# jcorsetti/oryon

Measured on AMD Instinct MI355X. Metric: image-pairs/sec end-to-end (feat+match+reg) @224², C=256; ADD(-S) parity, higher is better.
Workload: dtype f32

## Files before the change

oryon_amd/csrc/pdsc_encoder.hip:

```cpp
#include <stdlib.h>
#include "common.h"
#include "pdsc.h"
#include "pdsc_blocks.h"

namespace oryon {

__global__ __launch_bounds__(256) void pdsc_center_kernel(const float *__restrict__ src, const float *__restrict__ tgt,
                                                           const int32_t *__restrict__ n_rows, int n_cap,
                                                           float *__restrict__ corr_pos )
{
    __shared__ double s_part[4][6];
    __shared__ float s_mean[6];
    const int b = blockIdx.x, t = threadIdx.x, lane = t & 63, wave = t >> 6;
    const int n = n_rows[b];
    const float *s = src + (size_t)b * n_cap * 3, *g = tgt + (size_t)b * n_cap * 3;
    double acc[6] = {0, 0, 0, 0, 0, 0};
    for (int i = t; i < n; i += 256) {
#pragma unroll
        for (int d = 0; d < 3; ++d) { acc[d] += s[3 * i + d]; acc[3 + d] += g[3 * i + d]; }
    }
#pragma unroll
    for (int d = 0; d < 6; ++d) {
        double v = acc[d];
#pragma unroll
        for (int off = 32; off > 0; off >>= 1) v += __shfl_xor(v, off);
        if (lane == 0) s_part[wave][d] = v;
    }
    __syncthreads();
    if (t < 6) s_mean[t] = (float)((s_part[0][t] + s_part[1][t] + s_part[2][t] + s_part[3][t]) / (double)(n > 0 ? n : 1));
    __syncthreads();
    float *o = corr_pos + (size_t)b * n_cap * 8;
    for (int i = t; i < n_cap; i += 256) {
        float v[8];
#pragma unroll
        for (int d = 0; d < 3; ++d) {
            v[d] = i < n ? s[3 * i + d] - s_mean[d] : 0.0f;
            v[3 + d] = i < n ? g[3 * i + d] - s_mean[3 + d] : 0.0f;
        }
        v[6] = v[7] = 0.0f;
#pragma unroll
        for (int d = 0; d < 8; ++d) o[(size_t)i * 8 + d] = v[d];
    }
}

constexpr int LIN_ROWS = 64, LIN_COLS = 128, LIN_BK = 32, LIN_LD = LIN_BK + 1;

template <bool RELU, bool RESID>
__global__ __launch_bounds__(256) void pdsc_linear_kernel(const float *__restrict__ X, int ldx, size_t x_batch,
                                                           const float *__restrict__ W, const float *__restrict__ bias,
                                                           const float *__restrict__ R, int ldr, size_t r_batch,
                                                           float *__restrict__ Y, int ldy, size_t y_batch, int K, int N,
                                                           const int32_t *__restrict__ n_rows)
{
    __shared__ float Xs[LIN_ROWS * LIN_LD];
    __shared__ float Ws[LIN_COLS * LIN_LD];
    const int b = blockIdx.z;
    const int m0 = blockIdx.x * LIN_ROWS, n0 = blockIdx.y * LIN_COLS;
    if (n_rows && m0 >= n_rows[b]) return;
    const int t = threadIdx.x, lane = t & 63, wave = t >> 6;
    const int wm = wave >> 1, wn = wave & 1, l31 = lane & 31, hi = lane >> 5;
    const float *x = X + (size_t)b * x_batch + (size_t)m0 * ldx;
    f32x16 acc[2];
#pragma unroll
    for (int j = 0; j < 2; ++j)
#pragma unroll
        for (int r = 0; r < 16; ++r) acc[j][r] = 0.0f;

    for (int k0 = 0; k0 < K; k0 += LIN_BK) {
        constexpr int NX = (LIN_ROWS * LIN_BK) / 256, NW = (LIN_COLS * LIN_BK) / 256;
        float xv[NX], wv[NW];
#pragma unroll
        for (int i = 0; i < NX; ++i) {
            const int e = t + 256 * i, row = e >> 5, kk = e & 31;
            xv[i] = (k0 + kk < K) ? x[(size_t)row * ldx + k0 + kk] : 0.0f;
        }
#pragma unroll
        for (int i = 0; i < NW; ++i) {
            const int e = t + 256 * i, col = e >> 5, kk = e & 31;
            wv[i] = (n0 + col < N && k0 + kk < K) ? W[(size_t)(n0 + col) * K + k0 + kk] : 0.0f;
        }
        __syncthreads();
#pragma unroll
        for (int i = 0; i < NX; ++i) {
            const int e = t + 256 * i;
            Xs[(e >> 5) * LIN_LD + (e & 31)] = xv[i];
        }
#pragma unroll
        for (int i = 0; i < NW; ++i) {
            const int e = t + 256 * i;
            Ws[(e >> 5) * LIN_LD + (e & 31)] = wv[i];
        }
        __syncthreads();
        const float *xa = Xs + (wm * 32 + l31) * LIN_LD + hi;
        const float *wb = Ws + (wn * 64 + l31) * LIN_LD + hi;
#pragma unroll
        for (int ks = 0; ks < LIN_BK / 2; ++ks) {
            const float a = xa[2 * ks];
            acc[0] = __builtin_amdgcn_mfma_f32_32x32x2f32(a, wb[2 * ks], acc[0], 0, 0, 0);
            acc[1] = __builtin_amdgcn_mfma_f32_32x32x2f32(a, wb[32 * LIN_LD + 2 * ks], acc[1], 0, 0, 0);
        }
    }
#pragma unroll
    for (int j = 0; j < 2; ++j) {
        const int c = n0 + wn * 64 + j * 32 + l31;
        if (c >= N) continue;
        const float bv = bias ? bias[c] : 0.0f;
#pragma unroll
        for (int r = 0; r < 16; ++r) {
            const int row = m0 + wm * 32 + crow(r, hi);
            float v = acc[j][r] + bv;
            if (RELU) v = v > 0.0f ? v : 0.0f;
            if (RESID) v += R[(size_t)b * r_batch + (size_t)row * ldr + c];
            Y[(size_t)b * y_batch + (size_t)row * ldy + c] = v;
        }
    }
}

__global__ __launch_bounds__(256) void pdsc_sc_kernel(const float *__restrict__ src, const float *__restrict__ tgt,
                                                       const int32_t *__restrict__ n_rows, int n_cap, float inv_sigma2,
                                                       float *__restrict__ sc)
{
    const int b = blockIdx.z, kt = blockIdx.y;
    const int n = n_rows[b];
    const int t = threadIdx.x, lane = t & 63, wave = t >> 6, l31 = lane & 31, hi = lane >> 5;
    const int qb = blockIdx.x * 4 + wave;
    if (qb * 32 >= n || kt * ATT_KT >= n) return;
    const float *sp = src + (size_t)b * n_cap * 3, *tp = tgt + (size_t)b * n_cap * 3;
    const int q = qb * 32 + l31;
    float sq[3], tq[3];
#pragma unroll
    for (int d = 0; d < 3; ++d) { sq[d] = sp[(size_t)q * 3 + d]; tq[d] = tp[(size_t)q * 3 + d]; }
    float4 *out = reinterpret_cast<float4 *>(sc) + ((((size_t)b * (n_cap / 32) + qb) * (n_cap / ATT_KT) + kt) * 8) * 64 + lane;
#pragma unroll
    for (int v4 = 0; v4 < 8; ++v4) {
        float o[4];
#pragma unroll
        for (int e = 0; e < 4; ++e) {
            const int r = (v4 & 3) * 4 + e, kb = v4 >> 2;
            const int k = kt * ATT_KT + kb * 32 + crow(r, hi);
            float v = -1.0f;
            if (k < n) {
                const float dx = sq[0] - sp[(size_t)k * 3], dy = sq[1] - sp[(size_t)k * 3 + 1], dz = sq[2] - sp[(size_t)k * 3 + 2];
                const float ex = tq[0] - tp[(size_t)k * 3], ey = tq[1] - tp[(size_t)k * 3 + 1], ez = tq[2] - tp[(size_t)k * 3 + 2];
                const float ds = sqrt_rn(dx * dx + dy * dy + dz * dz);
                const float dt = sqrt_rn(ex * ex + ey * ey + ez * ez);
                const float df = ds - dt;
                v = 1.0f - df * df * inv_sigma2;
                v = v > 0.0f ? v : 0.0f;
            }
            o[e] = v;
        }
        out[(size_t)v4 * 64] = make_float4(o[0], o[1], o[2], o[3]);
    }
}

template <int C>
__global__ __launch_bounds__(256) void pdsc_attention_kernel(const float *__restrict__ QKV, const float *__restrict__ sc,
                                                              const int32_t *__restrict__ n_rows, int n_cap,
                                                              float inv_sqrt_c, float *__restrict__ msg,
                                                              int KS, float *__restrict__ part_o, float *__restrict__ part_ml)
{
    constexpr int LD = C + 4;
    constexpr int CB = C / 32;
    constexpr int F4_PER_ROW = C / 4, PER_THREAD = ATT_KT * F4_PER_ROW / 256;
    __shared__ __attribute__((aligned(16))) float Ks[ATT_KT * LD];
    __shared__ __attribute__((aligned(16))) float Vs[ATT_KT * LD];
    const int b = blockIdx.z, split = blockIdx.y;
    const int n = n_rows[b];
    const int q0 = blockIdx.x * ATT_Q;
    if (q0 >= n) return;
    const int n_tiles = (n + ATT_KT - 1) / ATT_KT, per = (n_tiles + KS - 1) / KS;
    const int j_begin = split * per * ATT_KT;
    const int j_end = ((split + 1) * per * ATT_KT < n) ? (split + 1) * per * ATT_KT : n;
    const int t = threadIdx.x, lane = t & 63, wave = t >> 6, l31 = lane & 31, hi = lane >> 5;
    const int qrow = q0 + wave * 32 + l31;
    const float *base = QKV + (size_t)b * n_cap * 3 * C;
    const float4 *sc_q = reinterpret_cast<const float4 *>(sc) + (((size_t)b * (n_cap / 32) + (q0 / 32 + wave)) * (n_cap / ATT_KT)) * 8 * 64 + lane;
    const bool q_live = q0 + wave * 32 < n;

    float4 kv[PER_THREAD], vv[PER_THREAD], scv[8];
    auto fetch = [&](int j0) {
#pragma unroll
        for (int i = 0; i < PER_THREAD; ++i) {
            const int e = t + 256 * i, row = e / F4_PER_ROW, c4 = e % F4_PER_ROW;
            const bool in = j0 + row < n_cap;
            const float *rp = base + (size_t)(in ? j0 + row : 0) * 3 * C;
            kv[i] = in ? *reinterpret_cast<const float4 *>(rp + C + 4 * c4) : make_float4(0.f, 0.f, 0.f, 0.f);
            vv[i] = in ? *reinterpret_cast<const float4 *>(rp + 2 * C + 4 * c4) : make_float4(0.f, 0.f, 0.f, 0.f);
        }
        const float4 *sp = sc_q + (size_t)(j0 / ATT_KT) * 8 * 64;
#pragma unroll
        for (int v4 = 0; v4 < 8; ++v4) scv[v4] = q_live ? sp[(size_t)v4 * 64] : make_float4(-1.f, -1.f, -1.f, -1.f);
    };
    auto land = [&]() {
#pragma unroll
        for (int i = 0; i < PER_THREAD; ++i) {
            const int e = t + 256 * i, row = e / F4_PER_ROW, c4 = e % F4_PER_ROW;
            *reinterpret_cast<float4 *>(Ks + row * LD + 4 * c4) = kv[i];
            *reinterpret_cast<float4 *>(Vs + row * LD + 4 * c4) = vv[i];
        }
    };

    float qreg[C / 2];
    {
        const float2 *qv = reinterpret_cast<const float2 *>(base + (size_t)qrow * 3 * C);
#pragma unroll
        for (int ks = 0; ks < C / 2; ++ks) {
            const float2 v = qv[ks];
            qreg[ks] = hi ? v.y : v.x;
        }
    }
    f32x16 acc_o[CB];
#pragma unroll
    for (int cb = 0; cb < CB; ++cb)
#pragma unroll
        for (int r = 0; r < 16; ++r) acc_o[cb][r] = 0.0f;
    float m_run = -INFINITY, l_run = 0.0f;

    if (j_begin < j_end) fetch(j_begin);
    for (int j0 = j_begin; j0 < j_end; j0 += ATT_KT) {
        __syncthreads();
        land();
        float4 sct[8];
#pragma unroll
        for (int v4 = 0; v4 < 8; ++v4) sct[v4] = scv[v4];
        __syncthreads();
        if (j0 + ATT_KT < j_end) fetch(j0 + ATT_KT);

        f32x16 s[2];
#pragma unroll
        for (int kb = 0; kb < 2; ++kb)
#pragma unroll
            for (int r = 0; r < 16; ++r) s[kb][r] = 0.0f;
        {
            const float *ka0 = Ks + l31 * LD + hi, *ka1 = Ks + (32 + l31) * LD + hi;
#pragma unroll
            for (int ks = 0; ks < C / 2; ++ks) {
                s[0] = __builtin_amdgcn_mfma_f32_32x32x2f32(ka0[2 * ks], qreg[ks], s[0], 0, 0, 0);
                s[1] = __builtin_amdgcn_mfma_f32_32x32x2f32(ka1[2 * ks], qreg[ks], s[1], 0, 0, 0);
            }
        }
        float m_tile = -INFINITY;
#pragma unroll
        for (int kb = 0; kb < 2; ++kb)
#pragma unroll
            for (int r = 0; r < 16; ++r) {
                const float4 q4 = sct[kb * 4 + (r >> 2)];
                const float scq = (r & 3) == 0 ? q4.x : (r & 3) == 1 ? q4.y : (r & 3) == 2 ? q4.z : q4.w;
                float v = scq * (s[kb][r] * inv_sqrt_c);
                v = (scq >= 0.0f) ? v : -INFINITY;
                s[kb][r] = v;
                m_tile = fmaxf(m_tile, v);
            }
        m_tile = fmaxf(m_tile, __shfl_xor(m_tile, 32));
        const float m_new = fmaxf(m_run, m_tile);
        const float alpha = __expf(m_run - m_new);
        float l_tile = 0.0f;
#pragma unroll
        for (int kb = 0; kb < 2; ++kb)
#pragma unroll
            for (int r = 0; r < 16; ++r) {
                const float p = expf(s[kb][r] - m_new);
                s[kb][r] = p;
                l_tile += p;
            }
        l_run = l_run * alpha + l_tile;
        m_run = m_new;
#pragma unroll
        for (int cb = 0; cb < CB; ++cb)
#pragma unroll
            for (int r = 0; r < 16; ++r) acc_o[cb][r] *= alpha;
#pragma unroll
        for (int kb = 0; kb < 2; ++kb)
#pragma unroll
            for (int r = 0; r < 16; ++r) {
                const float *va = Vs + (kb * 32 + crow(r, hi)) * LD + l31;
                const float p = s[kb][r];
#pragma unroll
                for (int cb = 0; cb < CB; ++cb) acc_o[cb] = __builtin_amdgcn_mfma_f32_32x32x2f32(va[cb * 32], p, acc_o[cb], 0, 0, 0);
            }
    }
    const float l_all = l_run + __shfl_xor(l_run, 32);
    if (KS > 1) {
        const size_t prow = ((size_t)split * gridDim.z + b) * n_cap + qrow;
        float *po = part_o + prow * C;
#pragma unroll
        for (int cb = 0; cb < CB; ++cb)
#pragma unroll
            for (int g = 0; g < 4; ++g) {
                float4 v;
                v.x = acc_o[cb][4 * g + 0]; v.y = acc_o[cb][4 * g + 1]; v.z = acc_o[cb][4 * g + 2]; v.w = acc_o[cb][4 * g + 3];
                *reinterpret_cast<float4 *>(po + cb * 32 + 8 * g + 4 * hi) = v;
            }
        if (hi == 0) { part_ml[prow * 2] = m_run; part_ml[prow * 2 + 1] = l_all; }
        return;
    }
// ... 1325 lines not shown
```

oryon_amd/csrc/pdsc_solver.hip:

```cpp
#include <stdlib.h>
#include "common.h"
#include "kabsch.h"
#include "pdsc.h"

namespace oryon {

__global__ __launch_bounds__(256) void pdsc_seed_keys_kernel(const float *__restrict__ src, const float *__restrict__ conf,
                                                              const int32_t *__restrict__ n_rows, int n_cap, float radius,
                                                              float *__restrict__ key)
{
    extern __shared__ float sm[];
    float *px = sm, *py = sm + n_cap, *pz = sm + 2 * n_cap, *sc = sm + 3 * n_cap;
    const int b = blockIdx.y, t = threadIdx.x;
    const int n = n_rows[b];
    if ((int)blockIdx.x * 64 >= n) return;
    for (int i = t; i < n; i += 256) {
        px[i] = src[((size_t)b * n_cap + i) * 3 + 0];
        py[i] = src[((size_t)b * n_cap + i) * 3 + 1];
        pz[i] = src[((size_t)b * n_cap + i) * 3 + 2];
        sc[i] = conf[(size_t)b * n_cap + i];
    }
    __syncthreads();
    const int i = blockIdx.x * 64 + (t >> 2), part = t & 3;
    bool lm = true;
// ... 323 lines not shown
        const float4 *fa = reinterpret_cast<const float4 *>(kf + a * (C + 4)), *fb = reinterpret_cast<const float4 *>(kf + c2 * (C + 4));
        for (int c4 = 0; c4 < C / 4; ++c4) {
            const float4 x = fa[c4], y = fb[c4];
            dot = fmaf(x.x, y.x, dot);
            dot = fmaf(x.y, y.y, dot);
            dot = fmaf(x.z, y.z, dot);
            dot = fmaf(x.w, y.w, dot);
        }
        float fm = 1.0f - (1.0f - dot) * inv_sigma2;
        fm = fm > 0.0f ? fm : 0.0f;
        const float *pa = kc + a * 6, *pb = kc + c2 * 6;
        const float dx = pa[0] - pb[0], dy = pa[1] - pb[1], dz = pa[2] - pb[2];
        const float ex = pa[3] - pb[3], ey = pa[4] - pb[4], ez = pa[5] - pb[5];
        const float df = sqrt_rn(dx * dx + dy * dy + dz * dz) - sqrt_rn(ex * ex + ey * ey + ez * ez);
        float smv = 1.0f - df * df * inv_sigma_d2;
        smv = smv > 0.0f ? smv : 0.0f;
        const float v = fm * smv;
        Mo[a * k_cfg + c2] = v;
        Mo[c2 * k_cfg + a] = v;
    }
}

__device__ __forceinline__ unsigned wave_min_u32(unsigned v)
{
#define ORYON_DPP_MIN(ctrl, rmask)                                                                                              \
    {                                                                                                                           \
        const unsigned o = (unsigned)__builtin_amdgcn_update_dpp((int)v, (int)v, ctrl, rmask, 0xf, false);                      \
        v = o < v ? o : v;                                                                                                      \
    }
    ORYON_DPP_MIN(0x111, 0xf)
    ORYON_DPP_MIN(0x112, 0xf)
    ORYON_DPP_MIN(0x114, 0xf)
    ORYON_DPP_MIN(0x118, 0xf)
    ORYON_DPP_MIN(0x142, 0xa)
    ORYON_DPP_MIN(0x143, 0xc)
#undef ORYON_DPP_MIN
    return (unsigned)__builtin_amdgcn_readlane((int)v, 63);
}

template <int C, int R>
__global__ __launch_bounds__(64) void pdsc_knn_wave_kernel(const float *__restrict__ feat_n, const float *__restrict__ src,
                                                            const float *__restrict__ tgt, const int32_t *__restrict__ n_rows, int n_cap,
                                                            const int32_t *__restrict__ n_seeds, int S_cap, int k_cfg, float inv_sigma2,
                                                            float inv_sigma_d2, int32_t *__restrict__ knn_out, float *__restrict__ M_out,
                                                            const float *__restrict__ dist_pre , int n_batch)
{
    extern __shared__ float sm[];
    const int lin = blockIdx.x + gridDim.x * blockIdx.y;
    const int b = (lin / 8 / (int)gridDim.x) * 8 + (lin & 7), s = (lin / 8) % (int)gridDim.x;
    if (b >= n_batch || s >= n_seeds[b]) return;
    const int n = n_rows[b];
    const int k = k_cfg < n - 1 ? k_cfg : n - 1;
    float *kf = sm;
    float *kc = kf + k_cfg * (C + 4);
    const int lane = threadIdx.x;
    const float *F = feat_n + (size_t)b * n_cap * C;
    const float *dp = dist_pre + ((size_t)b * S_cap + s) * n_cap;
    unsigned key[R];
    int rr[R];
#pragma unroll
    for (int r = 0; r < R; ++r) {
        const int j = lane + 64 * r;
        unsigned kx = 0xffffffffu;
        if (j < n) {
            const unsigned bits = __float_as_uint(dp[j]);
            kx = (bits >> 31) ? ~bits : (bits | 0x80000000u);
        }
        key[r] = kx;
        rr[r] = r;
    }
#pragma unroll
    for (int pass = 0; pass < R; ++pass) {
#pragma unroll
        for (int r = pass & 1; r + 1 < R; r += 2) {
            const bool sw = key[r] > key[r + 1];
            const unsigned ka = key[r], kb = key[r + 1];
            const int ra = rr[r], rb = rr[r + 1];
            key[r] = sw ? kb : ka; key[r + 1] = sw ? ka : kb;
            rr[r] = sw ? rb : ra;  rr[r + 1] = sw ? ra : rb;
        }
    }
    int mine = 0;
    for (int t = 0; t <= k; ++t) {
        const unsigned mk = wave_min_u32(key[0]);
        const unsigned cand = key[0] == mk ? (unsigned)(lane + 64 * rr[0]) : 0xffffffffu;
        const unsigned mi = wave_min_u32(cand);
        if (lane == (int)(mi & 63u)) {
#pragma unroll
            for (int r = 0; r + 1 < R; ++r) { key[r] = key[r + 1]; rr[r] = rr[r + 1]; }
            key[R - 1] = 0xffffffffu;
        }
        if (t >= 1 && lane == t - 1) mine = (int)mi;
    }
    if (lane < k) knn_out[((size_t)b * S_cap + s) * k_cfg + lane] = mine;
    static_assert(C == 128, "two channels per lane");
    for (int a = 0; a < k; ++a) {
        const int row = __shfl(mine, a);
        const float2 v = reinterpret_cast<const float2 *>(F + (size_t)row * C)[lane];
        *reinterpret_cast<float2 *>(kf + a * (C + 4) + 2 * lane) = v;
    }
    if (lane < k) {
#pragma unroll
        for (int d = 0; d < 3; ++d) {
            kc[lane * 6 + d] = src[((size_t)b * n_cap + mine) * 3 + d];
            kc[lane * 6 + 3 + d] = tgt[((size_t)b * n_cap + mine) * 3 + d];
        }
    }
    __syncthreads();
    float *Mo = M_out + ((size_t)b * S_cap + s) * k_cfg * k_cfg;
    for (int e = lane; e < k; e += 64) Mo[e * k_cfg + e] = 0.0f;
    const int n_pairs = k * (k - 1) / 2;
    for (int e = lane; e < n_pairs; e += 64) {
        int a = (int)((2.0f * k - 1.0f - sqrt_rn((2.0f * k - 1.0f) * (2.0f * k - 1.0f) - 8.0f * (float)e)) * 0.5f);
        while (a > 0 && a * (2 * k - a - 1) / 2 > e) --a;
        while ((a + 1) * (2 * k - a - 2) / 2 <= e) ++a;
        const int c2 = a + 1 + (e - a * (2 * k - a - 1) / 2);
        float dot = 0.0f;
        const float4 *fa = reinterpret_cast<const float4 *>(kf + a * (C + 4)), *fb = reinterpret_cast<const float4 *>(kf + c2 * (C + 4));
        for (int c4 = 0; c4 < C / 4; ++c4) {
            const float4 x = fa[c4], y = fb[c4];
            dot = fmaf(x.x, y.x, dot);
            dot = fmaf(x.y, y.y, dot);
            dot = fmaf(x.z, y.z, dot);
            dot = fmaf(x.w, y.w, dot);
        }
        float fm = 1.0f - (1.0f - dot) * inv_sigma2;
        fm = fm > 0.0f ? fm : 0.0f;
        const float *pa = kc + a * 6, *pb = kc + c2 * 6;
        const float dx = pa[0] - pb[0], dy = pa[1] - pb[1], dz = pa[2] - pb[2];
        const float ex = pa[3] - pb[3], ey = pa[4] - pb[4], ez = pa[5] - pb[5];
        const float df = sqrt_rn(dx * dx + dy * dy + dz * dz) - sqrt_rn(ex * ex + ey * ey + ez * ez);
        float smv = 1.0f - df * df * inv_sigma_d2;
        smv = smv > 0.0f ? smv : 0.0f;
        const float v = fm * smv;
        Mo[a * k_cfg + c2] = v;
        Mo[c2 * k_cfg + a] = v;
    }
}

constexpr int HYP_MAX_IT = 16;
__global__ __launch_bounds__(64) void pdsc_power_kernel(const int32_t *__restrict__ n_rows, const int32_t *__restrict__ n_seeds,
                                                         int S_cap, int k_cfg, int num_iterations, const float *__restrict__ Mmat,
                                                         float *__restrict__ v_hist ,
                                                         int32_t *__restrict__ close_hist )
{
    const int b = blockIdx.y, s = blockIdx.x, lane = threadIdx.x;
    if (s >= n_seeds[b]) return;
    const int n = n_rows[b];
    const int k = k_cfg < n - 1 ? k_cfg : n - 1;
    __shared__ float v_sh[KNN_MAX_K];
    float mrow[KNN_MAX_K];
    const float *Ms = Mmat + ((size_t)b * S_cap + s) * k_cfg * k_cfg;
#pragma unroll
    for (int c = 0; c < KNN_MAX_K; ++c) mrow[c] = (lane < k && c < k) ? Ms[lane * k_cfg + c] : 0.0f;
    float vl = 1.0f;
    for (int it = 0; it < num_iterations; ++it) {
        v_sh[lane] = vl;
        __syncthreads();
        float u = 0.0f;
#pragma unroll
        for (int c = 0; c < KNN_MAX_K; ++c)
            if (c < k) u = fmaf(mrow[c], v_sh[c], u);
        __syncthreads();
        if (lane >= k) u = 0.0f;
        float sq = u * u;
#pragma unroll
        for (int off = 32; off > 0; off >>= 1) sq += __shfl_xor(sq, off);
        const float vn = u / (sqrt_rn(sq) + 1e-6f);
        const bool close = (lane >= k) || (fabsf(vn - vl) <= 1e-8f + 1e-5f * fabsf(vl));
        const bool all = __all(close);
        const size_t h = ((size_t)b * S_cap + s) * num_iterations + it;
        v_hist[h * KNN_MAX_K + lane] = vn;
        if (lane == 0) close_hist[h] = all ? 1 : 0;
        vl = (lane < k) ? vn : 1.0f;
    }
}

__device__ __forceinline__ unsigned long long shfl_xor_u64(unsigned long long v, int m)
{
    const unsigned lo = (unsigned)__shfl_xor((int)(unsigned)v, m), hi = (unsigned)__shfl_xor((int)(unsigned)(v >> 32), m);
    return ((unsigned long long)hi << 32) | lo;
}
__device__ __forceinline__ unsigned long long bitonic_cx(unsigned long long x, int stride, bool keep_min)
{
    const unsigned long long p = shfl_xor_u64(x, stride);
    const bool lt = x < p;
    return (lt == keep_min) ? x : p;
}
__device__ __forceinline__ unsigned long long wave_sort64(unsigned long long x, int lane, bool desc)
{
#pragma unroll
    for (int size = 2; size <= 64; size <<= 1)
#pragma unroll
        for (int stride = size >> 1; stride > 0; stride >>= 1) {
            const bool up = (((lane & size) == 0) || size == 64) != desc;
            x = bitonic_cx(x, stride, ((lane & stride) == 0) == up);
        }
    return x;
}
__device__ __forceinline__ unsigned long long wave_merge64(unsigned long long x, int lane, bool desc)
{
#pragma unroll
    for (int stride = 32; stride > 0; stride >>= 1) x = bitonic_cx(x, stride, ((lane & stride) == 0) != desc);
    return x;
}

template <int EPT>
__global__ __launch_bounds__(256) void pdsc_hyp_fused_kernel(const float *__restrict__ feat_n, const float *__restrict__ src,
                                                              const float *__restrict__ tgt, const int32_t *__restrict__ n_rows, int n_cap,
                                                              const float *__restrict__ dist_pre ,
                                                              const int32_t *__restrict__ n_seeds,
                                                              int S_cap, int k_cfg, float inv_sigma2, float inv_sigma_d2,
                                                              int32_t *__restrict__ knn_out, float *__restrict__ M_out, int n_batch)
{
    constexpr int C = 128;
    static_assert(EPT == 2 || EPT == 4, "lists per wave");
    extern __shared__ float sm[];
    const int lin = blockIdx.x + gridDim.x * blockIdx.y;
    const int b = (lin / 8 / (int)gridDim.x) * 8 + (lin & 7), s = (lin / 8) % (int)gridDim.x;
    if (b >= n_batch || s >= n_seeds[b]) return;
    const int n = n_rows[b];
    const int k = k_cfg < n - 1 ? k_cfg : n - 1;
    unsigned long long *lists = reinterpret_cast<unsigned long long *>(sm);
    float *kf = sm + 512;
    float *kc = kf + k_cfg * (C + 4);
    int *kidx = reinterpret_cast<int *>(kc + k_cfg * 6);
    const int t = threadIdx.x, lane = t & 63, wave = t >> 6;
    const float *F = feat_n + (size_t)b * n_cap * C;
    const float *dp = dist_pre + ((size_t)b * S_cap + s) * n_cap;
    {
        unsigned long long x[EPT];
#pragma unroll
        for (int e = 0; e < EPT; ++e) {
            const int j = (wave * EPT + e) * 64 + lane;
            unsigned kx = 0xffffffffu;
            if (j < n) {
                const unsigned bits = __float_as_uint(dp[j]);
                kx = (bits >> 31) ? ~bits : (bits | 0x80000000u);
                kx = kx == 0xffffffffu ? 0xfffffffeu : kx;
            }
            x[e] = ((unsigned long long)kx << 32) | (unsigned)j;
        }
#pragma unroll
        for (int e = 0; e < EPT; ++e) x[e] = wave_sort64(x[e], lane, (e & 1) != 0);
        unsigned long long y;
        if constexpr (EPT == 4) {
            unsigned long long y0 = x[0] < x[1] ? x[0] : x[1], y1 = x[2] < x[3] ? x[2] : x[3];
            y0 = wave_merge64(y0, lane, false);
            y1 = wave_merge64(y1, lane, true);
            y = y0 < y1 ? y0 : y1;
        } else {
            y = x[0] < x[1] ? x[0] : x[1];
        }
        y = wave_merge64(y, lane, false);
        lists[wave * 64 + lane] = y;
        __syncthreads();
        if ((wave & 1) == 0) {
            const unsigned long long o = lists[(wave + 1) * 64 + 63 - lane];
            y = wave_merge64(y < o ? y : o, lane, false);
        }
        __syncthreads();
        if (wave == 2) lists[2 * 64 + lane] = y;
        __syncthreads();
        if (wave == 0) {
            const unsigned long long o = lists[2 * 64 + 63 - lane];
            y = wave_merge64(y < o ? y : o, lane, false);
            if (lane >= 1 && lane <= k) kidx[lane - 1] = (int)(unsigned)y;
        }
    }
    __syncthreads();
    for (int e = t; e < k * (C / 4); e += 256) {
        const int a = e / (C / 4), c4 = e % (C / 4);
        *reinterpret_cast<float4 *>(kf + a * (C + 4) + 4 * c4) = reinterpret_cast<const float4 *>(F + (size_t)kidx[a] * C)[c4];
    }
    for (int e = t; e < k * 3; e += 256) {
        const int a = e / 3, d = e % 3;
        kc[a * 6 + d] = src[((size_t)b * n_cap + kidx[a]) * 3 + d];
        kc[a * 6 + 3 + d] = tgt[((size_t)b * n_cap + kidx[a]) * 3 + d];
    }
    if (t < k) knn_out[((size_t)b * S_cap + s) * k_cfg + t] = kidx[t];
    __syncthreads();
    float *Mo = M_out + ((size_t)b * S_cap + s) * k_cfg * k_cfg;
    for (int e = t; e < k; e += 256) Mo[e * k_cfg + e] = 0.0f;
    const int n_pairs = k * (k - 1) / 2;
    for (int e = t; e < n_pairs; e += 256) {
        int a = (int)((2.0f * k - 1.0f - sqrt_rn((2.0f * k - 1.0f) * (2.0f * k - 1.0f) - 8.0f * (float)e)) * 0.5f);
        while (a > 0 && a * (2 * k - a - 1) / 2 > e) --a;
        while ((a + 1) * (2 * k - a - 2) / 2 <= e) ++a;
        const int c2 = a + 1 + (e - a * (2 * k - a - 1) / 2);
        float dot = 0.0f;
        const float4 *fa = reinterpret_cast<const float4 *>(kf + a * (C + 4)), *fb = reinterpret_cast<const float4 *>(kf + c2 * (C + 4));
#pragma unroll 8
        for (int c4 = 0; c4 < C / 4; ++c4) {
            const float4 x = fa[c4], y = fb[c4];
            dot = fmaf(x.x, y.x, dot);
            dot = fmaf(x.y, y.y, dot);
            dot = fmaf(x.z, y.z, dot);
            dot = fmaf(x.w, y.w, dot);
        }
        float fm = 1.0f - (1.0f - dot) * inv_sigma2;
        fm = fm > 0.0f ? fm : 0.0f;
        const float *pa = kc + a * 6, *pb = kc + c2 * 6;
        const float dx = pa[0] - pb[0], dy = pa[1] - pb[1], dz = pa[2] - pb[2];
        const float ex = pa[3] - pb[3], ey = pa[4] - pb[4], ez = pa[5] - pb[5];
        const float df = sqrt_rn(dx * dx + dy * dy + dz * dz) - sqrt_rn(ex * ex + ey * ey + ez * ez);
        float smv = 1.0f - df * df * inv_sigma_d2;
        smv = smv > 0.0f ? smv : 0.0f;
        const float v = fm * smv;
        Mo[a * k_cfg + c2] = v;
        Mo[c2 * k_cfg + a] = v;
    }
}

__global__ __launch_bounds__(64) void pdsc_seed_solve_kernel(const float *__restrict__ src, const float *__restrict__ tgt,
                                                              const int32_t *__restrict__ n_rows, int n_cap,
                                                              const int32_t *__restrict__ n_seeds, int S_cap, int k_cfg,
                                                              int num_iterations, float inlier_thr, const int32_t *__restrict__ knn,
                                                              const float *__restrict__ v_hist, const int32_t *__restrict__ close_hist,
                                                              float *__restrict__ seed_T, float *__restrict__ fitness)
{
    const int b = blockIdx.y, s = blockIdx.x, lane = threadIdx.x;
    const int S = n_seeds[b];
    if (s >= S) return;
    const int n = n_rows[b];
    const int k = k_cfg < n - 1 ? k_cfg : n - 1;
    int stop = num_iterations - 1;
    for (int it = 0; it < num_iterations; ++it) {
        int ok = 1;
        for (int q = lane; q < S; q += 64) ok &= close_hist[((size_t)b * S_cap + q) * num_iterations + it];
        if (__all(ok)) { stop = it; break; }
    }
    const float *sp = src + (size_t)b * n_cap * 3, *tp = tgt + (size_t)b * n_cap * 3;
    const float vv = lane < k ? v_hist[(((size_t)b * S_cap + s) * num_iterations + stop) * KNN_MAX_K + lane] : 0.0f;
    float sum = vv;
#pragma unroll
    for (int off = 32; off > 0; off >>= 1) sum += __shfl_xor(sum, off);
    float w = vv / (sum + 1e-6f);
    w = w < 0.0f ? 0.0f : w;
    KabschAcc acc;
    acc.clear();
    if (lane < k) {
        const int j = knn[((size_t)b * S_cap + s) * k_cfg + lane];
        acc.add(sp[3 * j], sp[3 * j + 1], sp[3 * j + 2], tp[3 * j], tp[3 * j + 1], tp[3 * j + 2], w);
    }
    acc.wave_reduce();
    float T[16];
    acc.solve(T);
    int cnt = 0;
    for (int j = lane; j < n; j += 64) {
        const float x = sp[3 * j], y = sp[3 * j + 1], z = sp[3 * j + 2];
        const float dx = (T[0] * x + T[1] * y + T[2] * z + T[3]) - tp[3 * j];
        const float dy = (T[4] * x + T[5] * y + T[6] * z + T[7]) - tp[3 * j + 1];
        const float dz = (T[8] * x + T[9] * y + T[10] * z + T[11]) - tp[3 * j + 2];
        cnt += (sqrt_rn(dx * dx + dy * dy + dz * dz) < inlier_thr) ? 1 : 0;
    }
#pragma unroll
    for (int off = 32; off > 0; off >>= 1) cnt += __shfl_xor(cnt, off);
    if (lane == 0) {
        fitness[(size_t)b * S_cap + s] = (float)cnt / (float)n;
#pragma unroll
        for (int i = 0; i < 16; ++i) seed_T[((size_t)b * S_cap + s) * 16 + i] = T[i];
    }
}

__global__ __launch_bounds__(256) void pdsc_seed_select_kernel(const float *__restrict__ src, const float *__restrict__ tgt,
                                                                const int32_t *__restrict__ n_rows, int n_cap,
                                                                const int32_t *__restrict__ n_seeds, int S_cap, float inlier_thr,
                                                                const float *__restrict__ seed_T, const float *__restrict__ fitness,
                                                                int32_t *__restrict__ best, float *__restrict__ T_best,
                                                                uint8_t *__restrict__ labels)
{
    __shared__ int s_best;
    const int b = blockIdx.x, t = threadIdx.x;
    const int n = n_rows[b], S = n_seeds[b];
    if (S <= 0) {
        if (t == 0) best[b] = -1;
        return;
    }
    if (t == 0) {
        int bi = 0;
        float bf = fitness[(size_t)b * S_cap];
        for (int s = 1; s < S; ++s) {
            const float f = fitness[(size_t)b * S_cap + s];
            if (f > bf) { bf = f; bi = s; }
        }
        s_best = bi;
        best[b] = bi;
    }
    __syncthreads();
    float T[16];
#pragma unroll
    for (int i = 0; i < 16; ++i) T[i] = seed_T[((size_t)b * S_cap + s_best) * 16 + i];
    if (t < 16) T_best[(size_t)b * 16 + t] = T[t];
    const float *sp = src + (size_t)b * n_cap * 3, *tp = tgt + (size_t)b * n_cap * 3;
    if (labels)
        for (int j = t; j < n_cap; j += 256) {
            uint8_t lab = 0;
            if (j < n) {
                const float x = sp[3 * j], y = sp[3 * j + 1], z = sp[3 * j + 2];
                const float dx = (T[0] * x + T[1] * y + T[2] * z + T[3]) - tp[3 * j];
                const float dy = (T[4] * x + T[5] * y + T[6] * z + T[7]) - tp[3 * j + 1];
                const float dz = (T[8] * x + T[9] * y + T[10] * z + T[11]) - tp[3 * j + 2];
                lab = (sqrt_rn(dx * dx + dy * dy + dz * dz) < inlier_thr) ? 1 : 0;
            }
            labels[(size_t)b * n_cap + j] = lab;
        }
}

__global__ __launch_bounds__(256) void pdsc_refine_kernel(const float *__restrict__ src, const float *__restrict__ tgt,
                                                           const int32_t *__restrict__ n_rows, int n_cap, float tau,
                                                           const float *__restrict__ T_in, const int32_t *__restrict__ status_in,
                                                           const int32_t *__restrict__ n_seeds, float *__restrict__ T_out,
                                                           int32_t *__restrict__ status_out)
{
    __shared__ float sT[16];
    __shared__ double s_red[4][17];
    __shared__ int s_cnt[4];
    const int b = blockIdx.x, t = threadIdx.x, lane = t & 63, wave = t >> 6;
    const int n = n_rows[b];
    int st = status_in ? status_in[b] : ORYON_PAIR_OK;
    if (st == ORYON_PAIR_OK && ((n_seeds && n_seeds[b] <= 0) || n < 2)) st = ORYON_PAIR_NO_CORR;
    if (st != ORYON_PAIR_OK) {
        if (t < 16) T_out[(size_t)b * 16 + t] = (t % 5 == 0) ? 1.0f : 0.0f;
        if (t == 0 && status_out) status_out[b] = st;
        return;
    }
    if (t < 16) sT[t] = T_in[(size_t)b * 16 + t];
    __syncthreads();
    const float *sp = src + (size_t)b * n_cap * 3, *tp = tgt + (size_t)b * n_cap * 3;
    int prev = 0;
    for (int it = 0; it < 20; ++it) {
        float T[12];
#pragma unroll
        for (int i = 0; i < 12; ++i) T[i] = sT[i];
        KabschAcc acc;
        acc.clear();
        int cnt = 0;
        for (int j = t; j < n; j += 256) {
            const float x = sp[3 * j], y = sp[3 * j + 1], z = sp[3 * j + 2];
            const float bx = tp[3 * j], by = tp[3 * j + 1], bz = tp[3 * j + 2];
            const float dx = (T[0] * x + T[1] * y + T[2] * z + T[3]) - bx;
            const float dy = (T[4] * x + T[5] * y + T[6] * z + T[7]) - by;
            const float dz = (T[8] * x + T[9] * y + T[10] * z + T[11]) - bz;
            const float d = sqrt_rn(dx * dx + dy * dy + dz * dz);
            if (d < tau) {
                ++cnt;
                const float q = d / tau;
                acc.add(x, y, z, bx, by, bz, 1.0f / (1.0f + q * q));
            }
        }
        acc.wave_reduce();
#pragma unroll
        for (int off = 32; off > 0; off >>= 1) cnt += __shfl_xor(cnt, off);
        __syncthreads();
        if (lane == 0) {
            s_cnt[wave] = cnt;
            s_red[wave][0] = acc.sw;
#pragma unroll
            for (int i = 0; i < 3; ++i) { s_red[wave][1 + i] = acc.sa[i]; s_red[wave][4 + i] = acc.sb[i]; }
#pragma unroll
            for (int i = 0; i < 9; ++i) s_red[wave][7 + i] = acc.sab[i];
        }
        __syncthreads();
// ... 114 lines not shown
```

Measured before the change: 24340.

## Stage key points in LDS, coalesce power-iteration loads, register-block pairwise feature dots

The spatial-consistency kernel now loads each key tile's source and target coordinates into shared memory once per block instead of every lane re-reading them from global memory. The power-iteration kernel reads the matrix column-wise (valid because it is symmetric) so the loads coalesce, and it skips the unused tail of the matvec in chunks of eight. The pairwise compatibility kernel replaces its per-pair triangular index decode with 2x2 tiles, so each thread computes four dot products from four shared feature rows and reuses each load. The tiling adds index-mapping complexity and edge cases for odd k, and the early return that now follows the barrier could hurt the coordinate staging.

```diff
diff --git a/oryon_amd/csrc/pdsc_encoder.hip b/oryon_amd/csrc/pdsc_encoder.hip
--- a/oryon_amd/csrc/pdsc_encoder.hip
+++ b/oryon_amd/csrc/pdsc_encoder.hip
@@ -124,8 +124,15 @@
     const int n = n_rows[b];
     const int t = threadIdx.x, lane = t & 63, wave = t >> 6, l31 = lane & 31, hi = lane >> 5;
     const int qb = blockIdx.x * 4 + wave;
-    if (qb * 32 >= n || kt * ATT_KT >= n) return;
+    if (kt * ATT_KT >= n) return;
     const float *sp = src + (size_t)b * n_cap * 3, *tp = tgt + (size_t)b * n_cap * 3;
+    __shared__ float ks[ATT_KT * 3], kq[ATT_KT * 3];
+    if (t < ATT_KT * 3) {
+        ks[t] = sp[(size_t)kt * ATT_KT * 3 + t];
+        kq[t] = tp[(size_t)kt * ATT_KT * 3 + t];
+    }
+    __syncthreads();
+    if (qb * 32 >= n) return;
     const int q = qb * 32 + l31;
     float sq[3], tq[3];
 #pragma unroll
@@ -137,11 +144,11 @@
 #pragma unroll
         for (int e = 0; e < 4; ++e) {
             const int r = (v4 & 3) * 4 + e, kb = v4 >> 2;
-            const int k = kt * ATT_KT + kb * 32 + crow(r, hi);
+            const int kl = kb * 32 + crow(r, hi), k = kt * ATT_KT + kl;
             float v = -1.0f;
             if (k < n) {
-                const float dx = sq[0] - sp[(size_t)k * 3], dy = sq[1] - sp[(size_t)k * 3 + 1], dz = sq[2] - sp[(size_t)k * 3 + 2];
-                const float ex = tq[0] - tp[(size_t)k * 3], ey = tq[1] - tp[(size_t)k * 3 + 1], ez = tq[2] - tp[(size_t)k * 3 + 2];
+                const float dx = sq[0] - ks[kl * 3], dy = sq[1] - ks[kl * 3 + 1], dz = sq[2] - ks[kl * 3 + 2];
+                const float ex = tq[0] - kq[kl * 3], ey = tq[1] - kq[kl * 3 + 1], ez = tq[2] - kq[kl * 3 + 2];
                 const float ds = sqrt_rn(dx * dx + dy * dy + dz * dz);
                 const float dt = sqrt_rn(ex * ex + ey * ey + ez * ez);
                 const float df = ds - dt;
diff --git a/oryon_amd/csrc/pdsc_solver.hip b/oryon_amd/csrc/pdsc_solver.hip
--- a/oryon_amd/csrc/pdsc_solver.hip
+++ b/oryon_amd/csrc/pdsc_solver.hip
@@ -499,15 +499,18 @@
     float mrow[KNN_MAX_K];
     const float *Ms = Mmat + ((size_t)b * S_cap + s) * k_cfg * k_cfg;
 #pragma unroll
-    for (int c = 0; c < KNN_MAX_K; ++c) mrow[c] = (lane < k && c < k) ? Ms[lane * k_cfg + c] : 0.0f;
+    for (int c = 0; c < KNN_MAX_K; ++c) mrow[c] = (lane < k && c < k) ? Ms[c * k_cfg + lane] : 0.0f;
     float vl = 1.0f;
     for (int it = 0; it < num_iterations; ++it) {
         v_sh[lane] = vl;
         __syncthreads();
         float u = 0.0f;
 #pragma unroll
-        for (int c = 0; c < KNN_MAX_K; ++c)
-            if (c < k) u = fmaf(mrow[c], v_sh[c], u);
+        for (int c0 = 0; c0 < KNN_MAX_K; c0 += 8)
+            if (c0 < k) {
+#pragma unroll
+                for (int c = c0; c < c0 + 8; ++c) u = fmaf(mrow[c], v_sh[c], u);
+            }
         __syncthreads();
         if (lane >= k) u = 0.0f;
         float sq = u * u;
@@ -629,33 +632,41 @@
     __syncthreads();
     float *Mo = M_out + ((size_t)b * S_cap + s) * k_cfg * k_cfg;
     for (int e = t; e < k; e += 256) Mo[e * k_cfg + e] = 0.0f;
-    const int n_pairs = k * (k - 1) / 2;
-    for (int e = t; e < n_pairs; e += 256) {
-        int a = (int)((2.0f * k - 1.0f - sqrt_rn((2.0f * k - 1.0f) * (2.0f * k - 1.0f) - 8.0f * (float)e)) * 0.5f);
-        while (a > 0 && a * (2 * k - a - 1) / 2 > e) --a;
-        while ((a + 1) * (2 * k - a - 2) / 2 <= e) ++a;
-        const int c2 = a + 1 + (e - a * (2 * k - a - 1) / 2);
-        float dot = 0.0f;
-        const float4 *fa = reinterpret_cast<const float4 *>(kf + a * (C + 4)), *fb = reinterpret_cast<const float4 *>(kf + c2 * (C + 4));
-#pragma unroll 8
-        for (int c4 = 0; c4 < C / 4; ++c4) {
-            const float4 x = fa[c4], y = fb[c4];
-            dot = fmaf(x.x, y.x, dot);
-            dot = fmaf(x.y, y.y, dot);
-            dot = fmaf(x.z, y.z, dot);
-            dot = fmaf(x.w, y.w, dot);
-        }
+    const int H = (k + 1) / 2, n_tiles = H * (H + 1) / 2;
+    auto put = [&](int i, int j2, float dot) {
         float fm = 1.0f - (1.0f - dot) * inv_sigma2;
         fm = fm > 0.0f ? fm : 0.0f;
-        const float *pa = kc + a * 6, *pb = kc + c2 * 6;
+        const float *pa = kc + i * 6, *pb = kc + j2 * 6;
         const float dx = pa[0] - pb[0], dy = pa[1] - pb[1], dz = pa[2] - pb[2];
         const float ex = pa[3] - pb[3], ey = pa[4] - pb[4], ez = pa[5] - pb[5];
         const float df = sqrt_rn(dx * dx + dy * dy + dz * dz) - sqrt_rn(ex * ex + ey * ey + ez * ez);
         float smv = 1.0f - df * df * inv_sigma_d2;
         smv = smv > 0.0f ? smv : 0.0f;
         const float v = fm * smv;
-        Mo[a * k_cfg + c2] = v;
-        Mo[c2 * k_cfg + a] = v;
+        Mo[i * k_cfg + j2] = v;
+        Mo[j2 * k_cfg + i] = v;
+    };
+    for (int e = t; e < n_tiles; e += 256) {
+        int a = 0, c = e;
+        while (c >= H - a) { c -= H - a; ++a; }
+        c += a;
+        const bool hi_a = a + H < k, hi_c = c + H < k;
+        const float4 *f0 = reinterpret_cast<const float4 *>(kf + a * (C + 4)), *f1 = reinterpret_cast<const float4 *>(kf + c * (C + 4));
+        const float4 *f2 = reinterpret_cast<const float4 *>(kf + (hi_a ? a + H : a) * (C + 4));
+        const float4 *f3 = reinterpret_cast<const float4 *>(kf + (hi_c ? c + H : c) * (C + 4));
+        float d01 = 0.0f, d23 = 0.0f, d03 = 0.0f, d12 = 0.0f;
+#pragma unroll 4
+        for (int c4 = 0; c4 < C / 4; ++c4) {
+            const float4 x0 = f0[c4], x1 = f1[c4], x2 = f2[c4], x3 = f3[c4];
+            d01 = fmaf(x0.x, x1.x, d01); d23 = fmaf(x2.x, x3.x, d23); d03 = fmaf(x0.x, x3.x, d03); d12 = fmaf(x1.x, x2.x, d12);
+            d01 = fmaf(x0.y, x1.y, d01); d23 = fmaf(x2.y, x3.y, d23); d03 = fmaf(x0.y, x3.y, d03); d12 = fmaf(x1.y, x2.y, d12);
+            d01 = fmaf(x0.z, x1.z, d01); d23 = fmaf(x2.z, x3.z, d23); d03 = fmaf(x0.z, x3.z, d03); d12 = fmaf(x1.z, x2.z, d12);
+            d01 = fmaf(x0.w, x1.w, d01); d23 = fmaf(x2.w, x3.w, d23); d03 = fmaf(x0.w, x3.w, d03); d12 = fmaf(x1.w, x2.w, d12);
+        }
+        if (a < c) put(a, c, d01);
+        if (a < c && hi_c) put(a + H, c + H, d23);
+        if (hi_c) put(a, c + H, d03);
+        if (a < c && hi_a) put(c, a + H, d12);
     }
 }
 
```

After: 24270. Within noise of the previous version (-0.3%).
